# alazarteka/Self-Forcing

Measured on AMD Instinct MI355X. Metric: decoded frames/sec/node, Wan-1.3B 832x480 4-step AR rollout, higher is better.
Workload: dtype bf16

## Files before the change

include/sf_hip.h:

```cpp
#ifndef SF_HIP_H
#define SF_HIP_H

#include <stddef.h>
#include <stdint.h>

#ifdef __cplusplus
extern "C" {
#endif

#define SF_HIP_ABI_VERSION 10

int sf_abi_version(void);
const char* sf_last_error(void);

enum sf_epilogue {
  SF_EPI_BIAS = 0,
  SF_EPI_BIAS_GELU = 1,
  SF_EPI_BIAS_RESID = 2,
  SF_EPI_BIAS_GATE_RESID = 3,
  SF_EPI_F32 = 4
};

typedef struct sf_gemm_args {
  const void* a;
  const void* w;
  const void* bias;
  void* out;
  const void* resid;
  const void* gate_mod;
  const void* gate_e0;
  int64_t gate_group_stride;
  int32_t rows_per_group;
  int32_t M, N, K;
  int32_t lda, ldw, ldo, ldr;
  int32_t epilogue;
  int32_t batch;
  int64_t a_bstride, w_bstride, o_bstride, r_bstride;
  int32_t structure;
} sf_gemm_args;

enum sf_gemm_structure { SF_GEMM_AUTO = 0, SF_GEMM_T128 = 1 ,
                         SF_GEMM_PP256 = 2 ,
                         SF_GEMM_PP128 = 3 ,
                         SF_GEMM_PP224 = 4, SF_GEMM_PP192 = 5  };

int sf_gemm_bf16(const sf_gemm_args* args, void* stream);

#define SF_FP8_AMAX_PARTS 1024
int sf_quantize_fp8(const void* x, int ldx, int M, int K, int rows_per_segment, void* q_out, float* scale_out, void* stream);

int sf_gemm_fp8(const sf_gemm_args* args, const float* a_scale, int rows_per_segment, const float* w_scale, void* stream);

int sf_small_linear_fp8(const void* x, const void* w_q, const float* w_scale, const void* bias, void* out, int M, int N, int K,
                        int rows_per_segment, int act_in, int act_out, void* stream);

int sf_small_linear(const void* x, const void* w, const void* bias, void* out, int M, int N, int K,
                    int act_in, int act_out, void* stream);

int sf_sinusoid_embedding(const void* t, int t_is_int64, void* out, int n, int dim, void* stream);

int sf_layernorm_modulate(const void* x, void* out, int M, int C, float eps, const void* mod_shift,
                          const void* mod_scale, const void* e0_shift, const void* e0_scale,
                          int64_t e0_group_stride, int rows_per_group, void* stream);

int sf_layernorm_affine(const void* x, const void* weight, const void* bias, void* out, int M, int C,
                        float eps, void* stream);

int sf_rmsnorm(const void* x, int ldx, const void* weight, void* out, int ldo, int M, int C, float eps,
               void* stream);

int sf_qkv_norm_rope_cache(const void* qkv, const void* norm_q_w, const void* norm_k_w, void* q_out,
                           void* k_cache, void* v_cache, const float* rope_cos, const float* rope_sin,
                           int B, int f, int h, int w, int C, int num_heads, int64_t cache_tokens,
                           int write_start, int start_frame, float eps, void* stream);

int sf_kv_evict(void* cache, int B, int64_t cache_tokens, int row_elems, int sink, int evict, int keep,
                void* scratch, size_t scratch_bytes, void* stream);

int sf_attention(const void* q, const void* k, const void* v, void* out, int B, int H, int Lq, int Lk,
// ... 267 lines not shown
```

self-forcing_amd/_lib.py:

```python
from __future__ import annotations

import ctypes as C
import os
import subprocess
from typing import Optional

os.environ.setdefault("ROC_SIGNAL_POOL_SIZE", "1024")

_HERE = os.path.dirname(os.path.abspath(__file__))
CSRC = os.path.join(_HERE, "csrc")
LIB_PATH = os.environ.get("SF_HIP_LIB") or os.path.join(CSRC, "libsf_hip.so")

ABI_VERSION = 10
FP8_AMAX_PARTS = 1024

EPI_BIAS, EPI_BIAS_GELU, EPI_BIAS_RESID, EPI_BIAS_GATE_RESID, EPI_F32 = 0, 1, 2, 3, 4
CONV_BIAS, CONV_BIAS_RESID, CONV_BIAS_CLAMP_F32 = 0, 1, 2
VAE_MAX_STAGES = 4
ACT_NONE, ACT_SILU, ACT_GELU = 0, 1, 2
ATTN_STRUCTURES = {"auto": 0, "r64": 1, "w8": 2, "w4": 3}
CONV_STRUCTURES = {"auto": 0, "igemm": 1, "halo": 2}
GEMM_STRUCTURES = {"auto": 0, "t128": 1, "pp256": 2, "pp128": 3, "pp224": 4, "pp192": 5}


class GemmArgs(C.Structure):
    _fields_ = [
        ("a", C.c_void_p), ("w", C.c_void_p), ("bias", C.c_void_p), ("out", C.c_void_p),
        ("resid", C.c_void_p), ("gate_mod", C.c_void_p), ("gate_e0", C.c_void_p),
        ("gate_group_stride", C.c_int64), ("rows_per_group", C.c_int32),
        ("M", C.c_int32), ("N", C.c_int32), ("K", C.c_int32),
        ("lda", C.c_int32), ("ldw", C.c_int32), ("ldo", C.c_int32), ("ldr", C.c_int32),
        ("epilogue", C.c_int32), ("batch", C.c_int32),
        ("a_bstride", C.c_int64), ("w_bstride", C.c_int64), ("o_bstride", C.c_int64), ("r_bstride", C.c_int64),
        ("structure", C.c_int32),
    ]


class LayerWeights(C.Structure):
    _fields_ = [(n, C.c_void_p) for n in (
        "modulation", "norm3_w", "norm3_b", "qkv_w", "qkv_b", "norm_q_w", "norm_k_w", "o_w", "o_b",
        "cq_w", "cq_b", "ckv_w", "ckv_b", "cnorm_q_w", "cnorm_k_w", "co_w", "co_b",
        "ffn0_w", "ffn0_b", "ffn2_w", "ffn2_b")]


class LayerFp8(C.Structure):
    _fields_ = [(n, C.c_void_p) for n in (
        "qkv_q", "o_q", "cq_q", "ckv_q", "co_q", "ffn0_q", "ffn2_q",
        "qkv_s", "o_s", "cq_s", "ckv_s", "co_s", "ffn0_s", "ffn2_s")]


FP8_MODEL_LINEARS = (("text0", ("text_embedding.0",)), ("text2", ("text_embedding.2",)), ("time0", ("time_embedding.0",)),
                     ("time2", ("time_embedding.2",)), ("tproj", ("time_projection.1",)), ("head", ("head.head",)),
                     ("pose", ("pose_proj",)))
FP8_LAYER_LINEARS = (("qkv", ("self_attn.q", "self_attn.k", "self_attn.v")), ("o", ("self_attn.o",)), ("cq", ("cross_attn.q",)),
                     ("ckv", ("cross_attn.k", "cross_attn.v")), ("co", ("cross_attn.o",)), ("ffn0", ("ffn.0",)), ("ffn2", ("ffn.2",)))
# ... 70 lines not shown
        ("head_gamma", C.c_void_p), ("head_conv", VaeConv),
    ]


class VaeEncoder(C.Structure):
    _fields_ = [
        ("z_dim", C.c_int32), ("n_stages", C.c_int32), ("res_per_stage", C.c_int32),
        ("temporal_down", C.c_int32 * VAE_MAX_STAGES),
        ("latent_mean", C.c_void_p), ("latent_std", C.c_void_p), ("conv1_w", C.c_void_p), ("conv1_b", C.c_void_p),
        ("in_conv", VaeConv), ("res_host", C.POINTER(VaeResBlock)),
        ("down_conv", VaeConv * VAE_MAX_STAGES), ("time_conv", VaeConv * VAE_MAX_STAGES),
        ("mid0", VaeResBlock), ("mid2", VaeResBlock),
        ("attn_gamma", C.c_void_p), ("attn_qk_w", C.c_void_p), ("attn_qk_b", C.c_void_p),
        ("attn_v_w", C.c_void_p), ("attn_v_b", C.c_void_p), ("attn_proj_w", C.c_void_p), ("attn_proj_b", C.c_void_p),
        ("head_gamma", C.c_void_p), ("head_conv", VaeConv),
    ]


class T5Layer(C.Structure):
    _fields_ = [(n, C.c_void_p) for n in ("norm1_w", "qk_w", "v_w", "o_w", "norm2_w", "gate_w", "fc1_w", "fc2_w", "pos_emb")]


class T5Model(C.Structure):
    _fields_ = ([(n, C.c_int32) for n in ("vocab", "dim", "dim_attn", "dim_ffn", "num_heads", "num_layers", "num_buckets")]
                + [("eps", C.c_float), ("token_embedding", C.c_void_p), ("layers_host", C.POINTER(T5Layer)),
                   ("final_norm_w", C.c_void_p)])


_vp, _i, _i64, _f, _sz = C.c_void_p, C.c_int, C.c_int64, C.c_float, C.c_size_t
SIGNATURES = {
    "sf_abi_version": (C.c_int, []),
    "sf_last_error": (C.c_char_p, []),
    "sf_gemm_bf16": (C.c_int, [C.POINTER(GemmArgs), _vp]),
    "sf_small_linear": (C.c_int, [_vp, _vp, _vp, _vp, _i, _i, _i, _i, _i, _vp]),
    "sf_quantize_fp8": (C.c_int, [_vp, _i, _i, _i, _i, _vp, _vp, _vp]),
    "sf_gemm_fp8": (C.c_int, [C.POINTER(GemmArgs), _vp, _i, _vp, _vp]),
    "sf_small_linear_fp8": (C.c_int, [_vp, _vp, _vp, _vp, _vp, _i, _i, _i, _i, _i, _i, _vp]),
    "sf_sinusoid_embedding": (C.c_int, [_vp, _i, _vp, _i, _i, _vp]),
    "sf_layernorm_modulate": (C.c_int, [_vp, _vp, _i, _i, _f, _vp, _vp, _vp, _vp, _i64, _i, _vp]),
    "sf_layernorm_affine": (C.c_int, [_vp, _vp, _vp, _vp, _i, _i, _f, _vp]),
    "sf_rmsnorm": (C.c_int, [_vp, _i, _vp, _vp, _i, _i, _i, _f, _vp]),
    "sf_qkv_norm_rope_cache": (C.c_int, [_vp, _vp, _vp, _vp, _vp, _vp, _vp, _vp, _i, _i, _i, _i, _i, _i, _i64,
                                         _i, _i, _f, _vp]),
    "sf_kv_evict": (C.c_int, [_vp, _i, _i64, _i, _i, _i, _i, _vp, _sz, _vp]),
    "sf_attention": (C.c_int, [_vp, _vp, _vp, _vp, _i, _i, _i, _i, _i64, _i64, _i64, _i64, _i64, _i64, _vp]),
    "sf_attention_ex": (C.c_int, [_vp, _vp, _vp, _vp, _i, _i, _i, _i, _i64, _i64, _i64, _i64, _i64, _i64, _i, _vp]),
    "sf_patchify": (C.c_int, [_vp, _vp, _i, _i, _i, _i, _i, _vp]),
    "sf_unpatchify_x0": (C.c_int, [_vp, _vp, _vp, _i, _vp, _vp, _i, _vp, _vp, _i, _i, _i, _i, _i, _i, _vp]),
    "sf_add_noise": (C.c_int, [_vp, _vp, _vp, _i, _vp, _vp, _i, _vp, _i, _i64, _vp]),
    "sf_lincomb_bf16": (C.c_int, [_vp, C.POINTER(C.c_void_p), C.POINTER(C.c_float), _i, _i64, _vp]),
    "sf_dit_workspace_bytes": (C.c_size_t, [C.POINTER(Model), _i, _i, _i, _i, _i]),
    "sf_dit_forward": (C.c_int, [C.POINTER(Model), C.POINTER(ForwardArgs), _vp]),
    "sf_dit_forward_pair": (C.c_int, [C.POINTER(Model), C.POINTER(ForwardArgs), C.POINTER(ForwardArgs), _vp]),
    "sf_conv_igemm": (C.c_int, [C.POINTER(ConvArgs), _vp]),
    "sf_conv_pick_nt": (C.c_int, [_i]),
    "sf_rmsnorm_silu_cl": (C.c_int, [_vp, _vp, _vp, _i64, _i, _i, _vp]),
    "sf_softmax_rows": (C.c_int, [_vp, _i64, _vp, _i64, _i, _i, _i, _f, _vp]),
    "sf_vae_prepare_latent": (C.c_int, [_vp, _vp, _vp, _vp, _vp, _vp, _i, _i, _i, _i, _vp]),
    "sf_vae_state_bytes": (C.c_size_t, [C.POINTER(VaeModel), _i, _i, _i]),
    "sf_vae_scratch_bytes": (C.c_size_t, [C.POINTER(VaeModel), _i, _i, _i]),
    "sf_vae_reset": (C.c_int, [C.POINTER(VaeModel), _vp, _sz, _i, _i, _i, _vp]),
    "sf_vae_decode_frames": (C.c_int, [C.POINTER(VaeModel), _vp, _sz, _vp, _sz, _vp, _i, _i, _i, _i, _i, _i, _i, _vp, _vp]),
    "sf_vae_prepare_pixels": (C.c_int, [_vp, _i, _i64, _vp, _i, _i, _i, _i, _vp]),
    "sf_vae_finish_latent": (C.c_int, [_vp, _i, _i, _vp, _i, _vp, _vp, _vp, _vp, _i, _i, _i, _i, _vp]),
    "sf_vae_encode_state_bytes": (C.c_size_t, [C.POINTER(VaeEncoder), _i, _i, _i]),
    "sf_vae_encode_scratch_bytes": (C.c_size_t, [C.POINTER(VaeEncoder), _i, _i, _i]),
# ... 57 lines not shown
```

self-forcing_amd/csrc/gemm_bf16.hip:

```cpp
#include <type_traits>
#include "sf_common.h"
#include "../../include/sf_hip.h"

namespace {

constexpr int BM = 128, BN = 128, BK = 64;
constexpr int GEMM_THREADS = 256;
constexpr int TILE_BYTES = BM * BK * 2;
constexpr int STAGE_BYTES = 2 * TILE_BYTES;
constexpr int GEMM_LDS = 2 * STAGE_BYTES;

struct GemmP {
  const bf16_t* a;
  const bf16_t* w;
  const bf16_t* bias;
  bf16_t* out;
  const bf16_t* resid;
  const bf16_t* gate_mod;
  const bf16_t* gate_e0;
  long gate_group_stride;
  int rows_per_group;
  int M, N, K, lda, ldw, ldo, ldr;
  int tiles_m, tiles_n;
  long a_bs, w_bs, o_bs, r_bs;
// ... 139 lines not shown
      if (m0 + i >= MT) break;
      const int m = min(m_base + (m0 + i) * 16 + r16, p.M - 1);
      const bf16_t* e0row = GATE ? p.gate_e0 + (long)(m / p.rows_per_group) * p.gate_group_stride : nullptr;
#pragma unroll
      for (int nt = 0; nt < 4; ++nt) {
        rv[i][nt] = RESID ? *reinterpret_cast<const bf16x4*>(p.resid + (long)m * p.ldr + ncol[nt]) : zero4;
        ge[i][nt] = GATE ? *reinterpret_cast<const bf16x4*>(e0row + ncol[nt]) : zero4;
      }
    }
#pragma unroll
    for (int i = 0; i < MB; ++i) {
      if (m0 + i >= MT) break;
      const int row = (m0 + i) * 16 + r16;
#pragma unroll
      for (int nt = 0; nt < 4; ++nt) {
        const int col = nt * 16 + cg * 4;
        const bf16x4 o = epi_math<EPI>(acc[m0 + i][nt], bias_v[nt], gm_v[nt], ge[i][nt], rv[i][nt]);
        const int chunk = (col >> 3) ^ (row & 7);
        *reinterpret_cast<bf16x4*>(wbuf + row * 128 + (chunk << 4) + (col & 4) * 2) = o;
      }
    }
  }
  __builtin_amdgcn_s_waitcnt(0xc07f);
  const int rr = lane >> 3, ch = lane & 7;
#pragma unroll
  for (int i = 0; i < 2 * MT; ++i) {
    const int row = i * 8 + rr;
    const int m = m_base + row, n = n_base + ch * 8;
    const bf16x8 v = *reinterpret_cast<const bf16x8*>(wbuf + row * 128 + ((ch ^ (row & 7)) << 4));
    if (m < p.M && n < p.N) *reinterpret_cast<bf16x8*>(p.out + (long)m * p.ldo + n) = v;
  }
}

template <int EPI, bool F8>
__global__ __launch_bounds__(GEMM_THREADS, 2) void gemm_bf16_kernel(GemmP p) {
  extern __shared__ __attribute__((aligned(16))) char smem[];
  const int tid = threadIdx.x;
  const int lane = tid & 63;
  const int wave = __builtin_amdgcn_readfirstlane(tid >> 6);

  if (blockIdx.y) {
    const long bz = blockIdx.y;
    p.a += bz * p.a_bs; p.w += bz * p.w_bs;
    if (EPI == SF_EPI_F32) p.out = reinterpret_cast<bf16_t*>(reinterpret_cast<float*>(p.out) + bz * p.o_bs); else p.out += bz * p.o_bs;
    if (p.resid) p.resid += bz * p.r_bs;
  }
  const int nwg = gridDim.x, bid = blockIdx.x;
  const int xcd = bid & 7, q8 = nwg >> 3, r8 = nwg & 7;
  const int wg = (xcd < r8 ? xcd * (q8 + 1) : r8 * (q8 + 1) + (xcd - r8) * q8) + (bid >> 3);
  constexpr int GROUP_M = 8;
  const int width = GROUP_M * p.tiles_n;
  const int group = wg / width, first_m = group * GROUP_M;
  const int gsz = min(p.tiles_m - first_m, GROUP_M);
  const int in_group = wg - group * width;
  const int tm = first_m + in_group % gsz, tn = in_group / gsz;
  const int m0 = tm * BM, n0 = tn * BN;

  const bf16_t* a_src[4];
  const bf16_t* w_src[4];
#pragma unroll
  for (int i = 0; i < 4; ++i) {
    const int r = (wave * 4 + i) * 8 + (lane >> 3);
    const int c = (lane & 7) ^ ((r >> 1) & 7);
    const int am = min(m0 + r, p.M - 1);
    const int wn = min(n0 + r, p.N - 1);
    a_src[i] = p.a + (long)am * p.lda + c * 8;
// ... 64 lines not shown
    for (int i = 0; i < 8; ++i) {
      const int mt = i >> 1, nt0 = (i & 1) * 2;
      acc[mt][nt0] = __builtin_amdgcn_mfma_f32_16x16x32_bf16(wf0[nt0], xf0[mt], acc[mt][nt0], 0, 0, 0);
      acc[mt][nt0 + 1] = __builtin_amdgcn_mfma_f32_16x16x32_bf16(wf0[nt0 + 1], xf0[mt], acc[mt][nt0 + 1], 0, 0, 0);
      if (i < 4) {
        xf1[i] = *reinterpret_cast<const bf16x8*>(buf + x_row_off + i * 2048 + coff1);
        glds16(a_src[i] + kn, sbase + i * 1024);
      } else {
        wf1[i - 4] = *reinterpret_cast<const bf16x8*>(buf + w_row_off + (i - 4) * 2048 + coff1);
        glds16(w_src[i - 4] + kn, sbase + TILE_BYTES + (i - 4) * 1024);
      }
      __builtin_amdgcn_sched_barrier(0);
    }
#pragma unroll
    for (int mt = 0; mt < 4; ++mt)
#pragma unroll
      for (int nt = 0; nt < 4; ++nt)
        acc[mt][nt] = __builtin_amdgcn_mfma_f32_16x16x32_bf16(wf1[nt], xf1[mt], acc[mt][nt], 0, 0, 0);
    __builtin_amdgcn_sched_barrier(0);
    __syncthreads();
  }

  if constexpr (F8) fp8_scale_acc<4>(p, acc, m0 + wr * 64, n0 + wc * 64, lane);
  const int mrow = m0 + wr * 64 + (lane & 15);
  const int ncol = n0 + wc * 64 + (lane >> 4) * 4;
  if (EPI != SF_EPI_F32 && (p.N & 7) == 0 && (p.ldo & 7) == 0)
    gemm_epilogue_lds<EPI, 4>(p, acc, m0 + wr * 64, n0 + wc * 64, smem + wave * 8192, lane);
  else
    gemm_epilogue<EPI, 4>(p, acc, mrow, ncol);
}


constexpr int PP_THREADS = 512;

template <int MT>
struct PPCfg {
  static constexpr int BM = 32 * MT;
  static constexpr int A_BYTES = BM * 128;
  static constexpr int B_BYTES = 256 * 128;
  static constexpr int STAGE = A_BYTES + B_BYTES;
  static constexpr int LDS = 2 * STAGE;
  static constexpr int PA = (2 * MT + 7) / 8;
};

template <int EPI, int MT, bool F8>
__global__ __launch_bounds__(PP_THREADS) void gemm_pp_kernel(GemmP p) {
  using Cfg = PPCfg<MT>;
  constexpr int BMp = Cfg::BM, PA = Cfg::PA;
  constexpr int HQA = (MT + 1) / 2, HQB = MT / 2;
  extern __shared__ __attribute__((aligned(16))) char smem[];
  const int tid = threadIdx.x;
  const int lane = tid & 63;
  const int wave = __builtin_amdgcn_readfirstlane(tid >> 6);
  const int grp = wave >> 2, wc = wave & 3;

  const int nwg = gridDim.x, bid = blockIdx.x;
  const int xcd = bid & 7, q8 = nwg >> 3, r8 = nwg & 7;
  const int wg = (xcd < r8 ? xcd * (q8 + 1) : r8 * (q8 + 1) + (xcd - r8) * q8) + (bid >> 3);
  constexpr int GROUP_M = MT >= 6 ? 4 : 8;
  const int width = GROUP_M * p.tiles_n;
  const int group = wg / width, first_m = group * GROUP_M;
  const int gsz = min(p.tiles_m - first_m, GROUP_M);
  const int in_group = wg - group * width;
  const int tm = first_m + in_group % gsz, tn = in_group / gsz;
  const int m0 = tm * BMp, n0 = tn * 256;

  const bf16_t* a_src[2][PA];
  const bf16_t* w_src[2][2];
#pragma unroll
  for (int h = 0; h < 2; ++h) {
#pragma unroll
    for (int i = 0; i < PA; ++i) {
      const int r = h * (BMp / 2) + (wave + 8 * i) * 8 + (lane >> 3);
      const int c = (lane & 7) ^ ((r >> 1) & 7);
      a_src[h][i] = p.a + (long)min(m0 + r, p.M - 1) * p.lda + c * 8;
    }
#pragma unroll
    for (int i = 0; i < 2; ++i) {
      const int r = h * 128 + (wave + 8 * i) * 8 + (lane >> 3);
      const int c = (lane & 7) ^ ((r >> 1) & 7);
      w_src[h][i] = p.w + (long)min(n0 + r, p.N - 1) * p.ldw + c * 8;
    }
  }
  auto dma_a = [&](int h, int kt) {
    char* base = smem + (kt & 1) * Cfg::STAGE + h * (Cfg::A_BYTES / 2) + wave * 1024;
#pragma unroll
    for (int i = 0; i < PA; ++i)
      if (wave + 8 * i < 2 * MT) glds16(a_src[h][i] + kt * BK, base + i * 8192);
  };
  auto dma_b = [&](int h, int kt) {
    char* base = smem + (kt & 1) * Cfg::STAGE + Cfg::A_BYTES + h * (Cfg::B_BYTES / 2) + wave * 1024;
#pragma unroll
    for (int i = 0; i < 2; ++i) glds16(w_src[h][i] + kt * BK, base + i * 8192);
  };

  const int i16 = lane & 15, kq = lane >> 4;
  const int swz = (i16 >> 1) & 7;
  const int x_row_off = (grp * (BMp / 2) + i16) * 128;
  const int w_row_off = Cfg::A_BYTES + (wc * 64 + i16) * 128;
  const int coff[2] = {((0 + kq) ^ swz) << 4, ((4 + kq) ^ swz) << 4};

  f32x4 acc[MT][4];
#pragma unroll
  for (int i = 0; i < MT; ++i)
#pragma unroll
    for (int j = 0; j < 4; ++j) acc[i][j] = f32x4{0.f, 0.f, 0.f, 0.f};
  bf16x8 af[HQA][2], bfr[4][2];

#ifdef SF_STAMP
  unsigned long long* stamp = (EPI == SF_EPI_BIAS && p.gate_e0) ? reinterpret_cast<unsigned long long*>(const_cast<bf16_t*>(p.gate_e0)) + ((long)bid * 2 + grp) * 8 : nullptr;
  if (stamp && (tid & 255) == 0) { stamp[0] = __builtin_amdgcn_s_memtime(); stamp[4] = __builtin_amdgcn_s_memrealtime(); }
#endif
  const int nk = p.K / BK;
  dma_a(0, 0); dma_a(1, 0); dma_b(0, 0); dma_b(1, 0);
  if (nk > 1) { dma_b(0, 1); dma_b(1, 1); asm volatile("s_waitcnt vmcnt(4)" ::: "memory"); }
  else asm volatile("s_waitcnt vmcnt(0)" ::: "memory");
  __builtin_amdgcn_s_barrier();
#ifdef SF_STAMP
  if (stamp && (tid & 255) == 0) stamp[1] = __builtin_amdgcn_s_memtime();
#endif
  if (grp == 1) __builtin_amdgcn_s_barrier();

  auto end_load_segment = [&]() {
    __builtin_amdgcn_s_waitcnt(0xc07f);
    __builtin_amdgcn_sched_barrier(0);
    __builtin_amdgcn_s_barrier();
    __builtin_amdgcn_sched_barrier(0);
  };
  auto cluster = [&](auto qc, int c0) {
    constexpr int q = decltype(qc)::value, NQ = q == 0 ? HQA : HQB;
    __builtin_amdgcn_s_setprio(1);
    if constexpr (F8) {
#pragma unroll
      for (int mt = 0; mt < NQ; ++mt)
#pragma unroll
        for (int nt = 0; nt < 2; ++nt)
          acc[q * HQA + mt][c0 + nt] = mfma_f8(bfr[c0 + nt][0], bfr[c0 + nt][1], af[mt][0], af[mt][1], acc[q * HQA + mt][c0 + nt]);
    } else {
#pragma unroll
      for (int ks = 0; ks < 2; ++ks)
#pragma unroll
        for (int mt = 0; mt < NQ; ++mt)
#pragma unroll
          for (int nt = 0; nt < 2; ++nt)
            acc[q * HQA + mt][c0 + nt] = __builtin_amdgcn_mfma_f32_16x16x32_bf16(bfr[c0 + nt][ks], af[mt][ks], acc[q * HQA + mt][c0 + nt], 0, 0, 0);
    }
    __builtin_amdgcn_s_setprio(0);
    __builtin_amdgcn_sched_barrier(0);
    __builtin_amdgcn_s_barrier();
    __builtin_amdgcn_sched_barrier(0);
  };
  auto read_a = [&](const char* buf, auto qc) {
    constexpr int q = decltype(qc)::value, NQ = q == 0 ? HQA : HQB;
#pragma unroll
    for (int mt = 0; mt < NQ; ++mt)
#pragma unroll
      for (int ks = 0; ks < 2; ++ks)
        af[mt][ks] = *reinterpret_cast<const bf16x8*>(buf + x_row_off + (q * HQA + mt) * 2048 + coff[ks]);
  };
  auto read_b = [&](const char* buf, int c0) {
#pragma unroll
    for (int nt = 0; nt < 2; ++nt)
#pragma unroll
      for (int ks = 0; ks < 2; ++ks)
        bfr[c0 + nt][ks] = *reinterpret_cast<const bf16x8*>(buf + w_row_off + (c0 + nt) * 2048 + coff[ks]);
  };

  constexpr std::integral_constant<int, 0> Q0{};
  constexpr std::integral_constant<int, 1> Q1{};
  for (int kt = 0; kt < nk; ++kt) {
    const char* buf = smem + (kt & 1) * Cfg::STAGE;
    const bool more1 = kt + 1 < nk, more2 = kt + 2 < nk;
    read_a(buf, Q0);
    read_b(buf, 0);
    if (more1) dma_a(0, kt + 1);
    end_load_segment();
    cluster(Q0, 0);
    read_b(buf, 2);
    if (more1) dma_a(1, kt + 1);
    end_load_segment();
    cluster(Q0, 2);
    read_a(buf, Q1);
    if (more2) dma_b(0, kt + 2);
    end_load_segment();
    cluster(Q1, 2);
    if (more2) {
      dma_b(1, kt + 2);
      asm volatile("s_waitcnt vmcnt(4)" ::: "memory");
    } else {
      asm volatile("s_waitcnt vmcnt(0)" ::: "memory");
    }
    end_load_segment();
    cluster(Q1, 0);
  }
  if (grp == 0) __builtin_amdgcn_s_barrier();
#ifdef SF_STAMP
  if (stamp && (tid & 255) == 0) stamp[2] = __builtin_amdgcn_s_memtime();
#endif

  const int m_base = m0 + grp * (BMp / 2), n_base = n0 + wc * 64;
  if constexpr (F8) fp8_scale_acc<MT>(p, acc, m_base, n_base, lane);
  if ((p.N & 7) == 0 && (p.ldo & 7) == 0)
    gemm_epilogue_lds<EPI, MT>(p, acc, m_base, n_base, smem + wave * (MT * 2048), lane);
  else
    gemm_epilogue<EPI, MT>(p, acc, m_base + (lane & 15), n_base + (lane >> 4) * 4);
#ifdef SF_STAMP
  asm volatile("s_waitcnt vmcnt(0)" ::: "memory");
  if (stamp && (tid & 255) == 0) { stamp[3] = __builtin_amdgcn_s_memtime(); stamp[5] = __builtin_amdgcn_s_memrealtime(); }
#endif
}

constexpr int PP2_A = 128 * 128, PP2_B = 256 * 128;
constexpr int PP2_LDS = 3 * (PP2_A + PP2_B);

template <int EPI, bool F8>
__global__ __launch_bounds__(PP_THREADS) void gemm_pp2_kernel(GemmP p) {
  extern __shared__ __attribute__((aligned(16))) char smem[];
  const int tid = threadIdx.x;
  const int lane = tid & 63;
  const int wave = __builtin_amdgcn_readfirstlane(tid >> 6);
  const int grp = wave >> 2, wc = wave & 3;

  const int nwg = gridDim.x, bid = blockIdx.x;
  const int xcd = bid & 7, q8 = nwg >> 3, r8 = nwg & 7;
  const int wg = (xcd < r8 ? xcd * (q8 + 1) : r8 * (q8 + 1) + (xcd - r8) * q8) + (bid >> 3);
  constexpr int GROUP_M = 8;
  const int width = GROUP_M * p.tiles_n;
  const int group = wg / width, first_m = group * GROUP_M;
  const int gsz = min(p.tiles_m - first_m, GROUP_M);
  const int in_group = wg - group * width;
  const int tm = first_m + in_group % gsz, tn = in_group / gsz;
  const int m0 = tm * 128, n0 = tn * 256;

  const bf16_t* a_src[2];
  const bf16_t* w_src[4];
#pragma unroll
  for (int i = 0; i < 2; ++i) {
    const int r = (wave + 8 * i) * 8 + (lane >> 3);
    a_src[i] = p.a + (long)min(m0 + r, p.M - 1) * p.lda + ((lane & 7) ^ ((r >> 1) & 7)) * 8;
  }
#pragma unroll
  for (int i = 0; i < 4; ++i) {
// ... 95 lines not shown

  const int m_base = m0 + grp * 64, n_base = n0 + wc * 64;
  if constexpr (F8) fp8_scale_acc<4>(p, acc, m_base, n_base, lane);
  if ((p.N & 7) == 0 && (p.ldo & 7) == 0)
    gemm_epilogue_lds<EPI, 4>(p, acc, m_base, n_base, smem + wave * 8192, lane);
  else
    gemm_epilogue<EPI, 4>(p, acc, m_base + (lane & 15), n_base + (lane >> 4) * 4);
}

template <int EPI, bool F8>
int launch_pp2(GemmP& p, hipStream_t s) {
  static bool attr = false;
  if (!attr) {
    (void)hipFuncSetAttribute(reinterpret_cast<const void*>(&gemm_pp2_kernel<EPI, F8>), hipFuncAttributeMaxDynamicSharedMemorySize, PP2_LDS);
    attr = true;
  }
  p.tiles_m = (p.M + 127) / 128;
  p.tiles_n = (p.N + 255) / 256;
  hipLaunchKernelGGL((gemm_pp2_kernel<EPI, F8>), dim3(p.tiles_m * p.tiles_n), dim3(PP_THREADS), PP2_LDS, s, p);
  return 0;
}

template <bool F8>
int launch_pp2_epi(GemmP& p, int epilogue, hipStream_t s) {
  switch (epilogue) {
    case SF_EPI_BIAS: return launch_pp2<SF_EPI_BIAS, F8>(p, s);
    case SF_EPI_BIAS_GELU: return launch_pp2<SF_EPI_BIAS_GELU, F8>(p, s);
    case SF_EPI_BIAS_RESID: return launch_pp2<SF_EPI_BIAS_RESID, F8>(p, s);
    case SF_EPI_BIAS_GATE_RESID: return launch_pp2<SF_EPI_BIAS_GATE_RESID, F8>(p, s);
    default: return -1;
  }
}

template <int EPI, int MT, bool F8>
int launch_pp(GemmP& p, hipStream_t s) {
  using Cfg = PPCfg<MT>;
  static bool attr = false;
  if (!attr) {
    (void)hipFuncSetAttribute(reinterpret_cast<const void*>(&gemm_pp_kernel<EPI, MT, F8>), hipFuncAttributeMaxDynamicSharedMemorySize, Cfg::LDS);
    attr = true;
  }
  p.tiles_m = (p.M + Cfg::BM - 1) / Cfg::BM;
  p.tiles_n = (p.N + 255) / 256;
  hipLaunchKernelGGL((gemm_pp_kernel<EPI, MT, F8>), dim3(p.tiles_m * p.tiles_n), dim3(PP_THREADS), Cfg::LDS, s, p);
  return 0;
}

template <int MT, bool F8>
int launch_pp_epi(GemmP& p, int epilogue, hipStream_t s) {
  switch (epilogue) {
    case SF_EPI_BIAS: return launch_pp<SF_EPI_BIAS, MT, F8>(p, s);
    case SF_EPI_BIAS_GELU: return launch_pp<SF_EPI_BIAS_GELU, MT, F8>(p, s);
    case SF_EPI_BIAS_RESID: return launch_pp<SF_EPI_BIAS_RESID, MT, F8>(p, s);
    case SF_EPI_BIAS_GATE_RESID: return launch_pp<SF_EPI_BIAS_GATE_RESID, MT, F8>(p, s);
    default: return -1;
  }
}

int check_args(const sf_gemm_args* a, const char* name, int bk) {
  SF_CHECK(a != nullptr, "%s: null args", name);
  SF_CHECK(a->M > 0 && a->N > 0 && a->K > 0, "%s: empty problem M=%d N=%d K=%d", name, a->M, a->N, a->K);
  SF_CHECK(a->K % bk == 0, "%s: K=%d must be a multiple of %d", name, a->K, bk);
  SF_CHECK(a->N % 4 == 0, "%s: N=%d must be a multiple of 4", name, a->N);
  SF_CHECK(a->lda % (bk / 8) == 0 && a->ldw % (bk / 8) == 0 && a->ldo % 4 == 0, "%s: lda/ldw must be multiples of %d, ldo of 4", name, bk / 8);
  SF_CHECK(a->lda >= a->K && a->ldw >= a->K && a->ldo >= a->N, "%s: leading dimension too small", name);
  SF_CHECK(a->a && a->w && a->out, "%s: null tensor", name);
  SF_CHECK(((uintptr_t)a->a % 16 == 0) && ((uintptr_t)a->w % 16 == 0) && ((uintptr_t)a->out % 8 == 0), "%s: misaligned tensor", name);
  if (a->epilogue == SF_EPI_BIAS_RESID || a->epilogue == SF_EPI_BIAS_GATE_RESID) {
    SF_CHECK(a->resid != nullptr && a->ldr >= a->N && a->ldr % 4 == 0, "%s: residual epilogue needs resid/ldr", name);
  }
  if (a->epilogue == SF_EPI_BIAS_GATE_RESID) {
    SF_CHECK(a->gate_mod && a->gate_e0 && a->rows_per_group > 0, "%s: gate epilogue needs gate_mod/gate_e0/rows_per_group", name);
  }
  SF_CHECK(a->structure >= SF_GEMM_AUTO && a->structure <= SF_GEMM_PP192, "%s: unknown structure %d", name, a->structure);
  return 0;
}

template <bool F8>
int run_gemm(const sf_gemm_args* a, GemmP& p, const char* name, hipStream_t s) {
  int st = a->structure;
  const int nk = p.K / BK;
  const bool pp_ok = a->batch <= 1 && a->epilogue != SF_EPI_F32 && nk >= 2;
  if (st == SF_GEMM_AUTO) {
    st = SF_GEMM_T128;
    if (pp_ok && a->M >= 1024 && a->N >= 1024 && a->K >= 512) {
      static const struct { int st, rows; double rel; } cand[] = {
          {SF_GEMM_PP256, 256, 1.00}, {SF_GEMM_PP224, 224, 1.02}, {SF_GEMM_PP192, 192, 1.05}, {SF_GEMM_PP128, 128, 1.14}};
      const long tn = (a->N + 255) / 256;
      double best = 1e30;
      for (const auto& c : cand) {
        const long tiles = (long)((a->M + c.rows - 1) / c.rows) * tn;
        const double cost = (double)((tiles + 255) / 256) * (c.rows / 256.0 * c.rel + 0.04);
        if (cost < best - 1e-9) { best = cost; st = c.st; }
      }
    }
  }
  const bool is_pp = st == SF_GEMM_PP256 || st == SF_GEMM_PP224 || st == SF_GEMM_PP192 || st == SF_GEMM_PP128;
  if (is_pp && !pp_ok) st = SF_GEMM_T128;
  else if (is_pp) {
    const int rc = st == SF_GEMM_PP256 ? launch_pp_epi<8, F8>(p, a->epilogue, s)
                 : st == SF_GEMM_PP224 ? launch_pp_epi<7, F8>(p, a->epilogue, s)
                 : st == SF_GEMM_PP192 ? launch_pp_epi<6, F8>(p, a->epilogue, s) : launch_pp2_epi<F8>(p, a->epilogue, s);
    SF_CHECK(rc == 0, "%s: unknown epilogue %d", name, a->epilogue);
    SF_HIP_LAUNCH_CHECK(name);
    return 0;
  }
  const int batch = a->batch > 1 ? a->batch : 1;
  p.a_bs = a->a_bstride; p.w_bs = a->w_bstride; p.o_bs = a->o_bstride; p.r_bs = a->r_bstride;
  SF_CHECK(batch == 1 || (a->a_bstride % 8 == 0 && a->w_bstride % 8 == 0 && a->o_bstride % 4 == 0 && a->r_bstride % 4 == 0),
           "%s: batch strides must keep 16-byte (operands) / 8-byte (output) alignment", name);
  const dim3 grid(p.tiles_m * p.tiles_n, batch), block(GEMM_THREADS);
  switch (a->epilogue) {
    case SF_EPI_BIAS: hipLaunchKernelGGL((gemm_bf16_kernel<SF_EPI_BIAS, F8>), grid, block, GEMM_LDS, s, p); break;
    case SF_EPI_BIAS_GELU: hipLaunchKernelGGL((gemm_bf16_kernel<SF_EPI_BIAS_GELU, F8>), grid, block, GEMM_LDS, s, p); break;
    case SF_EPI_BIAS_RESID: hipLaunchKernelGGL((gemm_bf16_kernel<SF_EPI_BIAS_RESID, F8>), grid, block, GEMM_LDS, s, p); break;
    case SF_EPI_BIAS_GATE_RESID: hipLaunchKernelGGL((gemm_bf16_kernel<SF_EPI_BIAS_GATE_RESID, F8>), grid, block, GEMM_LDS, s, p); break;
    case SF_EPI_F32:
      if constexpr (F8) {
        SF_CHECK(false, "%s: the raw fp32 epilogue is bf16-only", name);
      } else {
        SF_CHECK((uintptr_t)a->out % 16 == 0, "%s: fp32 output must be 16-byte aligned", name);
        hipLaunchKernelGGL((gemm_bf16_kernel<SF_EPI_F32, false>), grid, block, GEMM_LDS, s, p);
      }
      break;
    default: SF_CHECK(false, "%s: unknown epilogue %d", name, a->epilogue);
  }
  SF_HIP_LAUNCH_CHECK(name);
  return 0;
}

void fill_params(const sf_gemm_args* a, GemmP& p, int unit) {
  p.a = (const bf16_t*)a->a; p.w = (const bf16_t*)a->w; p.bias = (const bf16_t*)a->bias;
  p.out = (bf16_t*)a->out; p.resid = (const bf16_t*)a->resid;
  p.gate_mod = (const bf16_t*)a->gate_mod; p.gate_e0 = (const bf16_t*)a->gate_e0;
  p.gate_group_stride = a->gate_group_stride; p.rows_per_group = a->rows_per_group;
  p.M = a->M; p.N = a->N; p.K = a->K / unit; p.lda = a->lda / unit; p.ldw = a->ldw / unit; p.ldo = a->ldo; p.ldr = a->ldr;
  p.tiles_n = (a->N + BN - 1) / BN;
  p.tiles_m = (a->M + BM - 1) / BM;
  p.a_scale = nullptr; p.w_scale = nullptr; p.rows_per_seg = 1;
}

}

extern "C" int sf_gemm_bf16(const sf_gemm_args* a, void* stream) {
  if (const int rc = check_args(a, "sf_gemm_bf16", BK)) return rc;
  GemmP p;
  fill_params(a, p, 1);
  return run_gemm<false>(a, p, "sf_gemm_bf16", (hipStream_t)stream);
}

extern "C" int sf_gemm_fp8(const sf_gemm_args* a, const float* a_scale, int rows_per_segment, const float* w_scale, void* stream) {
  if (const int rc = check_args(a, "sf_gemm_fp8", 2 * BK)) return rc;
  SF_CHECK(a->batch <= 1, "sf_gemm_fp8: batched products are bf16-only");
  SF_CHECK(a_scale && w_scale && rows_per_segment > 0, "sf_gemm_fp8: needs a_scale, w_scale and rows_per_segment > 0");
  SF_CHECK((uintptr_t)w_scale % 16 == 0, "sf_gemm_fp8: w_scale must be 16-byte aligned");
  GemmP p;
  fill_params(a, p, 2);
  p.a_scale = a_scale; p.w_scale = w_scale; p.rows_per_seg = rows_per_segment;
  return run_gemm<true>(a, p, "sf_gemm_fp8", (hipStream_t)stream);
}
```

Before: 96.18.

## Add persistent tile-loop PP GEMM that prefetches next tile during epilogue

Adds a persistent variant of the ping-pong GEMM kernel that launches at most 256 workgroups and loops over output tiles. Each workgroup issues the first loads for its next tile before running the current tile's epilogue, which goes through separate LDS scratch regions. Stores are left outstanding and waited on with adjusted vmcnt counts. This is meant to hide epilogue and tile-startup latency and avoid extra waves when the tile count exceeds the grid. The cost is a larger LDS footprint, more complex counter-based synchronisation, and a serial tile walk per workgroup. Auto-selection switches to the loop form whenever the chosen PP config has more than 256 tiles.

New measurement: 97.07 (median of 6 runs). No clear change (+0.9%).

```diff
diff --git a/include/sf_hip.h b/include/sf_hip.h
--- a/include/sf_hip.h
+++ b/include/sf_hip.h
@@ -42,9 +42,12 @@
 enum sf_gemm_structure { SF_GEMM_AUTO = 0, SF_GEMM_T128 = 1 ,
                          SF_GEMM_PP256 = 2 ,
                          SF_GEMM_PP128 = 3 ,
-                         SF_GEMM_PP224 = 4, SF_GEMM_PP192 = 5  };
+                         SF_GEMM_PP224 = 4, SF_GEMM_PP192 = 5 ,
+                         SF_GEMM_PP256_LOOP = 6, SF_GEMM_PP224_LOOP = 7, SF_GEMM_PP192_LOOP = 8  };
 
 int sf_gemm_bf16(const sf_gemm_args* args, void* stream);
+
+int sf_gemm_pp_loop_lds_map(int row_tiles, int32_t out[7]);
 
 #define SF_FP8_AMAX_PARTS 1024
 int sf_quantize_fp8(const void* x, int ldx, int M, int K, int rows_per_segment, void* q_out, float* scale_out, void* stream);
diff --git a/self-forcing_amd/_lib.py b/self-forcing_amd/_lib.py
--- a/self-forcing_amd/_lib.py
+++ b/self-forcing_amd/_lib.py
@@ -20,7 +20,8 @@
 ACT_NONE, ACT_SILU, ACT_GELU = 0, 1, 2
 ATTN_STRUCTURES = {"auto": 0, "r64": 1, "w8": 2, "w4": 3}
 CONV_STRUCTURES = {"auto": 0, "igemm": 1, "halo": 2}
-GEMM_STRUCTURES = {"auto": 0, "t128": 1, "pp256": 2, "pp128": 3, "pp224": 4, "pp192": 5}
+GEMM_STRUCTURES = {"auto": 0, "t128": 1, "pp256": 2, "pp128": 3, "pp224": 4, "pp192": 5,
+                   "pp256_loop": 6, "pp224_loop": 7, "pp192_loop": 8}
 
 
 class GemmArgs(C.Structure):
@@ -157,6 +158,7 @@
     "sf_abi_version": (C.c_int, []),
     "sf_last_error": (C.c_char_p, []),
     "sf_gemm_bf16": (C.c_int, [C.POINTER(GemmArgs), _vp]),
+    "sf_gemm_pp_loop_lds_map": (C.c_int, [_i, C.POINTER(C.c_int32)]),
     "sf_small_linear": (C.c_int, [_vp, _vp, _vp, _vp, _i, _i, _i, _i, _i, _vp]),
     "sf_quantize_fp8": (C.c_int, [_vp, _i, _i, _i, _i, _vp, _vp, _vp]),
     "sf_gemm_fp8": (C.c_int, [C.POINTER(GemmArgs), _vp, _i, _vp, _vp]),
diff --git a/self-forcing_amd/csrc/gemm_bf16.hip b/self-forcing_amd/csrc/gemm_bf16.hip
--- a/self-forcing_amd/csrc/gemm_bf16.hip
+++ b/self-forcing_amd/csrc/gemm_bf16.hip
@@ -195,6 +195,74 @@
   }
 }
 
+template <int EPI, int MT, class RequestNext>
+__device__ __forceinline__ void gemm_epilogue_lds_loop(const GemmP& p, f32x4 (&acc)[MT][4], const bf16x4 (&bias_v)[4], int m_base, int n_base,
+                                                       char* wbuf, int lane, RequestNext&& request_next) {
+  const int r16 = lane & 15, cg = lane >> 4;
+  constexpr bool GATE = EPI == SF_EPI_BIAS_GATE_RESID;
+  constexpr bool RESID = EPI == SF_EPI_BIAS_RESID || EPI == SF_EPI_BIAS_GATE_RESID;
+  constexpr int HALF = 8 * MT;
+  constexpr int SPLIT = (MT + 1) / 2;
+  const bf16x4 zero4 = {(bf16_t)0.f, (bf16_t)0.f, (bf16_t)0.f, (bf16_t)0.f};
+  int ncol[4];
+  bf16x4 gm_v[4];
+#pragma unroll
+  for (int nt = 0; nt < 4; ++nt) {
+    ncol[nt] = min(n_base + nt * 16 + cg * 4, p.N - 4);
+    gm_v[nt] = GATE ? *reinterpret_cast<const bf16x4*>(p.gate_mod + ncol[nt]) : zero4;
+  }
+  bf16x4 rv[MT][4], ge[MT][4];
+  auto load_rows = [&](auto lo, auto hi) {
+#pragma unroll
+    for (int mt = decltype(lo)::value; mt < decltype(hi)::value; ++mt) {
+      const int m = min(m_base + mt * 16 + r16, p.M - 1);
+      const bf16_t* e0row = GATE ? p.gate_e0 + (long)(m / p.rows_per_group) * p.gate_group_stride : nullptr;
+#pragma unroll
+      for (int nt = 0; nt < 4; ++nt) {
+        rv[mt][nt] = RESID ? *reinterpret_cast<const bf16x4*>(p.resid + (long)m * p.ldr + ncol[nt]) : zero4;
+        ge[mt][nt] = GATE ? *reinterpret_cast<const bf16x4*>(e0row + ncol[nt]) : zero4;
+      }
+    }
+  };
+  constexpr std::integral_constant<int, 0> I0{};
+  constexpr std::integral_constant<int, SPLIT> IS{};
+  constexpr std::integral_constant<int, MT> IM{};
+  if (!GATE) load_rows(I0, IM);
+#pragma unroll
+  for (int nt = 0; nt < 4; ++nt) asm volatile("" ::"v"(bias_v[nt]));
+  request_next();
+  const int rr = lane >> 3, ch = lane & 7;
+#pragma unroll
+  for (int ps = 0; ps < 2; ++ps) {
+    if (GATE) {
+      if (ps == 0) load_rows(I0, IS); else load_rows(IS, IM);
+    }
+#pragma unroll
+    for (int mt = ps * (MT / 2); mt < (ps == 0 ? SPLIT : MT); ++mt) {
+      const int srow = mt * 16 + r16 - ps * HALF;
+#pragma unroll
+      for (int nt = 0; nt < 4; ++nt) {
+        const int col = nt * 16 + cg * 4;
+        const bf16x4 o = epi_math<EPI>(acc[mt][nt], bias_v[nt], gm_v[nt], ge[mt][nt], rv[mt][nt]);
+        const int chunk = (col >> 3) ^ (srow & 7);
+        if ((unsigned)srow < (unsigned)HALF) *reinterpret_cast<bf16x4*>(wbuf + srow * 128 + (chunk << 4) + (col & 4) * 2) = o;
+      }
+    }
+    __builtin_amdgcn_s_waitcnt(0xc07f);
+    bf16x8 v[MT];
+#pragma unroll
+    for (int i = 0; i < MT; ++i) {
+      const int srow = i * 8 + rr;
+      v[i] = *reinterpret_cast<const bf16x8*>(wbuf + srow * 128 + ((ch ^ (srow & 7)) << 4));
+    }
+#pragma unroll
+    for (int i = 0; i < MT; ++i) {
+      const int m = m_base + ps * HALF + i * 8 + rr, n = n_base + ch * 8;
+      if (m < p.M && n < p.N) *reinterpret_cast<bf16x8*>(p.out + (long)m * p.ldo + n) = v[i];
+    }
+  }
+}
+
 template <int EPI, bool F8>
 __global__ __launch_bounds__(GEMM_THREADS, 2) void gemm_bf16_kernel(GemmP p) {
   extern __shared__ __attribute__((aligned(16))) char smem[];
@@ -325,6 +393,8 @@
 
 
 constexpr int PP_THREADS = 512;
+constexpr int PP_LOOP_WGS = 256;
+constexpr bool PP_AUTO_TILE_LOOP = true;
 
 template <int MT>
 struct PPCfg {
@@ -334,9 +404,11 @@
   static constexpr int STAGE = A_BYTES + B_BYTES;
   static constexpr int LDS = 2 * STAGE;
   static constexpr int PA = (2 * MT + 7) / 8;
+  static constexpr int SCRATCH = MT * 1024;
+  static constexpr int LDS_LOOP = LDS + 4 * SCRATCH;
 };
 
-template <int EPI, int MT, bool F8>
+template <int EPI, int MT, bool F8, bool LOOP>
 __global__ __launch_bounds__(PP_THREADS) void gemm_pp_kernel(GemmP p) {
   using Cfg = PPCfg<MT>;
   constexpr int BMp = Cfg::BM, PA = Cfg::PA;
@@ -347,34 +419,43 @@
   const int wave = __builtin_amdgcn_readfirstlane(tid >> 6);
   const int grp = wave >> 2, wc = wave & 3;
 
-  const int nwg = gridDim.x, bid = blockIdx.x;
-  const int xcd = bid & 7, q8 = nwg >> 3, r8 = nwg & 7;
-  const int wg = (xcd < r8 ? xcd * (q8 + 1) : r8 * (q8 + 1) + (xcd - r8) * q8) + (bid >> 3);
+  const int nwg = LOOP ? p.tiles_m * p.tiles_n : gridDim.x, bid = blockIdx.x;
   constexpr int GROUP_M = MT >= 6 ? 4 : 8;
-  const int width = GROUP_M * p.tiles_n;
-  const int group = wg / width, first_m = group * GROUP_M;
-  const int gsz = min(p.tiles_m - first_m, GROUP_M);
-  const int in_group = wg - group * width;
-  const int tm = first_m + in_group % gsz, tn = in_group / gsz;
-  const int m0 = tm * BMp, n0 = tn * 256;
+  int m0, n0;
+  auto tile_origin = [&](int t) {
+    const int xcd = t & 7, q8 = nwg >> 3, r8 = nwg & 7;
+    const int wg = (xcd < r8 ? xcd * (q8 + 1) : r8 * (q8 + 1) + (xcd - r8) * q8) + (t >> 3);
+    const int width = GROUP_M * p.tiles_n;
+    const int group = wg / width, first_m = group * GROUP_M;
+    const int gsz = min(p.tiles_m - first_m, GROUP_M);
+    const int in_group = wg - group * width;
+    m0 = (first_m + in_group % gsz) * BMp;
+    n0 = (in_group / gsz) * 256;
+  };
 
   const bf16_t* a_src[2][PA];
   const bf16_t* w_src[2][2];
-#pragma unroll
-  for (int h = 0; h < 2; ++h) {
-#pragma unroll
-    for (int i = 0; i < PA; ++i) {
-      const int r = h * (BMp / 2) + (wave + 8 * i) * 8 + (lane >> 3);
-      const int c = (lane & 7) ^ ((r >> 1) & 7);
-      a_src[h][i] = p.a + (long)min(m0 + r, p.M - 1) * p.lda + c * 8;
-    }
-#pragma unroll
-    for (int i = 0; i < 2; ++i) {
-      const int r = h * 128 + (wave + 8 * i) * 8 + (lane >> 3);
-      const int c = (lane & 7) ^ ((r >> 1) & 7);
-      w_src[h][i] = p.w + (long)min(n0 + r, p.N - 1) * p.ldw + c * 8;
-    }
-  }
+  auto set_sources = [&]() {
+    int ln = lane;
+    if (LOOP) asm volatile("" : "+v"(ln));
+#pragma unroll
+    for (int h = 0; h < 2; ++h) {
+#pragma unroll
+      for (int i = 0; i < PA; ++i) {
+        const int r = h * (BMp / 2) + (wave + 8 * i) * 8 + (ln >> 3);
+        const int c = (ln & 7) ^ ((r >> 1) & 7);
+        a_src[h][i] = p.a + (long)min(m0 + r, p.M - 1) * p.lda + c * 8;
+      }
+#pragma unroll
+      for (int i = 0; i < 2; ++i) {
+        const int r = h * 128 + (wave + 8 * i) * 8 + (ln >> 3);
+        const int c = (ln & 7) ^ ((r >> 1) & 7);
+        w_src[h][i] = p.w + (long)min(n0 + r, p.N - 1) * p.ldw + c * 8;
+      }
+    }
+  };
+  tile_origin(bid);
+  set_sources();
   auto dma_a = [&](int h, int kt) {
     char* base = smem + (kt & 1) * Cfg::STAGE + h * (Cfg::A_BYTES / 2) + wave * 1024;
 #pragma unroll
@@ -385,6 +466,11 @@
     char* base = smem + (kt & 1) * Cfg::STAGE + Cfg::A_BYTES + h * (Cfg::B_BYTES / 2) + wave * 1024;
 #pragma unroll
     for (int i = 0; i < 2; ++i) glds16(w_src[h][i] + kt * BK, base + i * 8192);
+  };
+  const int nk = p.K / BK;
+  auto first_requests = [&]() {
+    dma_a(0, 0); dma_a(1, 0); dma_b(0, 0); dma_b(1, 0);
+    if (nk > 1) { dma_b(0, 1); dma_b(1, 1); }
   };
 
   const int i16 = lane & 15, kq = lane >> 4;
@@ -394,25 +480,13 @@
   const int coff[2] = {((0 + kq) ^ swz) << 4, ((4 + kq) ^ swz) << 4};
 
   f32x4 acc[MT][4];
-#pragma unroll
-  for (int i = 0; i < MT; ++i)
-#pragma unroll
-    for (int j = 0; j < 4; ++j) acc[i][j] = f32x4{0.f, 0.f, 0.f, 0.f};
   bf16x8 af[HQA][2], bfr[4][2];
 
 #ifdef SF_STAMP
   unsigned long long* stamp = (EPI == SF_EPI_BIAS && p.gate_e0) ? reinterpret_cast<unsigned long long*>(const_cast<bf16_t*>(p.gate_e0)) + ((long)bid * 2 + grp) * 8 : nullptr;
-  if (stamp && (tid & 255) == 0) { stamp[0] = __builtin_amdgcn_s_memtime(); stamp[4] = __builtin_amdgcn_s_memrealtime(); }
+  if (!LOOP && stamp && (tid & 255) == 0) { stamp[0] = __builtin_amdgcn_s_memtime(); stamp[4] = __builtin_amdgcn_s_memrealtime(); }
 #endif
-  const int nk = p.K / BK;
-  dma_a(0, 0); dma_a(1, 0); dma_b(0, 0); dma_b(1, 0);
-  if (nk > 1) { dma_b(0, 1); dma_b(1, 1); asm volatile("s_waitcnt vmcnt(4)" ::: "memory"); }
-  else asm volatile("s_waitcnt vmcnt(0)" ::: "memory");
-  __builtin_amdgcn_s_barrier();
-#ifdef SF_STAMP
-  if (stamp && (tid & 255) == 0) stamp[1] = __builtin_amdgcn_s_memtime();
-#endif
-  if (grp == 1) __builtin_amdgcn_s_barrier();
+  first_requests();
 
   auto end_load_segment = [&]() {
     __builtin_amdgcn_s_waitcnt(0xc07f);
@@ -461,46 +535,105 @@
 
   constexpr std::integral_constant<int, 0> Q0{};
   constexpr std::integral_constant<int, 1> Q1{};
-  for (int kt = 0; kt < nk; ++kt) {
-    const char* buf = smem + (kt & 1) * Cfg::STAGE;
-    const bool more1 = kt + 1 < nk, more2 = kt + 2 < nk;
-    read_a(buf, Q0);
-    read_b(buf, 0);
-    if (more1) dma_a(0, kt + 1);
-    end_load_segment();
-    cluster(Q0, 0);
-    read_b(buf, 2);
-    if (more1) dma_a(1, kt + 1);
-    end_load_segment();
-    cluster(Q0, 2);
-    read_a(buf, Q1);
-    if (more2) dma_b(0, kt + 2);
-    end_load_segment();
-    cluster(Q1, 2);
-    if (more2) {
-      dma_b(1, kt + 2);
-      asm volatile("s_waitcnt vmcnt(4)" ::: "memory");
+  constexpr int NST = 2 * MT;
+  const int ntiles = nwg;
+  bool stores_pending = false;
+  for (int tile = bid;;) {
+#ifdef SF_STAMP
+    const bool stamp_on = stamp && (tid & 255) == 0 && (!LOOP || tile == bid + (int)gridDim.x);
+    if (LOOP && stamp_on) { stamp[0] = __builtin_amdgcn_s_memtime(); stamp[4] = __builtin_amdgcn_s_memrealtime(); }
+#endif
+#pragma unroll
+    for (int i = 0; i < MT; ++i)
+#pragma unroll
+      for (int j = 0; j < 4; ++j) acc[i][j] = f32x4{0.f, 0.f, 0.f, 0.f};
+    if (LOOP && stores_pending) {
+      if (nk > 1) asm volatile("s_waitcnt vmcnt(%0)" ::"n"(4 + NST) : "memory");
+      else asm volatile("s_waitcnt vmcnt(%0)" ::"n"(NST) : "memory");
     } else {
-      asm volatile("s_waitcnt vmcnt(0)" ::: "memory");
-    }
-    end_load_segment();
-    cluster(Q1, 0);
-  }
-  if (grp == 0) __builtin_amdgcn_s_barrier();
+      if (nk > 1) asm volatile("s_waitcnt vmcnt(4)" ::: "memory");
+      else asm volatile("s_waitcnt vmcnt(0)" ::: "memory");
+    }
+    __builtin_amdgcn_s_barrier();
 #ifdef SF_STAMP
-  if (stamp && (tid & 255) == 0) stamp[2] = __builtin_amdgcn_s_memtime();
+    if (stamp_on) stamp[1] = __builtin_amdgcn_s_memtime();
 #endif
-
-  const int m_base = m0 + grp * (BMp / 2), n_base = n0 + wc * 64;
-  if constexpr (F8) fp8_scale_acc<MT>(p, acc, m_base, n_base, lane);
-  if ((p.N & 7) == 0 && (p.ldo & 7) == 0)
-    gemm_epilogue_lds<EPI, MT>(p, acc, m_base, n_base, smem + wave * (MT * 2048), lane);
-  else
-    gemm_epilogue<EPI, MT>(p, acc, m_base + (lane & 15), n_base + (lane >> 4) * 4);
+    if (grp == 1) __builtin_amdgcn_s_barrier();
+    bf16x4 bias_v[4];
+    if constexpr (LOOP) {
+#pragma unroll
+      for (int nt = 0; nt < 4; ++nt) {
+        bias_v[nt] = bf16x4{(bf16_t)0.f, (bf16_t)0.f, (bf16_t)0.f, (bf16_t)0.f};
+        if (p.bias) bias_v[nt] = *reinterpret_cast<const bf16x4*>(p.bias + min(n0 + wc * 64 + nt * 16 + (lane >> 4) * 4, p.N - 4));
+      }
+    }
+
+    for (int kt = 0; kt < nk; ++kt) {
+      const char* buf = smem + (kt & 1) * Cfg::STAGE;
+      const bool more1 = kt + 1 < nk, more2 = kt + 2 < nk;
+      read_a(buf, Q0);
+      read_b(buf, 0);
+      if (more1) dma_a(0, kt + 1);
+      end_load_segment();
+      cluster(Q0, 0);
+      read_b(buf, 2);
+      if (more1) dma_a(1, kt + 1);
+      end_load_segment();
+      cluster(Q0, 2);
+      read_a(buf, Q1);
+      if (more2) dma_b(0, kt + 2);
+      end_load_segment();
+      cluster(Q1, 2);
+      if (more2) {
+        dma_b(1, kt + 2);
+        asm volatile("s_waitcnt vmcnt(4)" ::: "memory");
+      } else {
+        asm volatile("s_waitcnt vmcnt(0)" ::: "memory");
+      }
+      end_load_segment();
+      cluster(Q1, 0);
+    }
+    if (grp == 0) __builtin_amdgcn_s_barrier();
 #ifdef SF_STAMP
-  asm volatile("s_waitcnt vmcnt(0)" ::: "memory");
-  if (stamp && (tid & 255) == 0) { stamp[3] = __builtin_amdgcn_s_memtime(); stamp[5] = __builtin_amdgcn_s_memrealtime(); }
+    if (stamp_on) stamp[2] = __builtin_amdgcn_s_memtime();
 #endif
+
+    const int m_base = m0 + grp * (BMp / 2), n_base = n0 + wc * 64;
+    if constexpr (F8) fp8_scale_acc<MT>(p, acc, m_base, n_base, lane);
+    if constexpr (!LOOP) {
+      if ((p.N & 7) == 0 && (p.ldo & 7) == 0)
+        gemm_epilogue_lds<EPI, MT>(p, acc, m_base, n_base, smem + wave * (MT * 2048), lane);
+      else
+        gemm_epilogue<EPI, MT>(p, acc, m_base + (lane & 15), n_base + (lane >> 4) * 4);
+    } else {
+      const int next = tile + gridDim.x;
+      auto request_next = [&]() {
+        __builtin_amdgcn_sched_barrier(0);
+        if (next < ntiles) {
+          tile_origin(next);
+          set_sources();
+          first_requests();
+        }
+        __builtin_amdgcn_sched_barrier(0);
+      };
+      char* scratch = smem + (grp == 0 ? Cfg::STAGE : 2 * Cfg::STAGE) + wc * Cfg::SCRATCH;
+      if ((p.N & 7) == 0 && (p.ldo & 7) == 0) {
+        gemm_epilogue_lds_loop<EPI, MT>(p, acc, bias_v, m_base, n_base, scratch, lane, request_next);
+        stores_pending = m_base + 16 * MT <= p.M && n_base + 64 <= p.N;
+      } else {
+        request_next();
+        gemm_epilogue<EPI, MT>(p, acc, m_base + (lane & 15), n_base + (lane >> 4) * 4);
+        stores_pending = false;
+      }
+    }
+#ifdef SF_STAMP
+    if (!LOOP) asm volatile("s_waitcnt vmcnt(0)" ::: "memory");
+    if (stamp_on) { stamp[3] = __builtin_amdgcn_s_memtime(); stamp[5] = __builtin_amdgcn_s_memrealtime(); }
+#endif
+    if (!LOOP) break;
+    tile += gridDim.x;
+    if (tile >= ntiles) break;
+  }
 }
 
 constexpr int PP2_A = 128 * 128, PP2_B = 256 * 128;
@@ -662,27 +795,30 @@
   }
 }
 
-template <int EPI, int MT, bool F8>
+template <int EPI, int MT, bool F8, bool LOOP>
 int launch_pp(GemmP& p, hipStream_t s) {
   using Cfg = PPCfg<MT>;
+  constexpr int lds = LOOP ? Cfg::LDS_LOOP : Cfg::LDS;
+  static_assert(lds <= 160 * 1024, "a workgroup's LDS");
   static bool attr = false;
   if (!attr) {
-    (void)hipFuncSetAttribute(reinterpret_cast<const void*>(&gemm_pp_kernel<EPI, MT, F8>), hipFuncAttributeMaxDynamicSharedMemorySize, Cfg::LDS);
+    (void)hipFuncSetAttribute(reinterpret_cast<const void*>(&gemm_pp_kernel<EPI, MT, F8, LOOP>), hipFuncAttributeMaxDynamicSharedMemorySize, lds);
     attr = true;
   }
   p.tiles_m = (p.M + Cfg::BM - 1) / Cfg::BM;
   p.tiles_n = (p.N + 255) / 256;
-  hipLaunchKernelGGL((gemm_pp_kernel<EPI, MT, F8>), dim3(p.tiles_m * p.tiles_n), dim3(PP_THREADS), Cfg::LDS, s, p);
+  const int tiles = p.tiles_m * p.tiles_n;
+  hipLaunchKernelGGL((gemm_pp_kernel<EPI, MT, F8, LOOP>), dim3(LOOP ? min(tiles, PP_LOOP_WGS) : tiles), dim3(PP_THREADS), lds, s, p);
   return 0;
 }
 
-template <int MT, bool F8>
+template <int MT, bool F8, bool LOOP>
 int launch_pp_epi(GemmP& p, int epilogue, hipStream_t s) {
   switch (epilogue) {
-    case SF_EPI_BIAS: return launch_pp<SF_EPI_BIAS, MT, F8>(p, s);
-    case SF_EPI_BIAS_GELU: return launch_pp<SF_EPI_BIAS_GELU, MT, F8>(p, s);
-    case SF_EPI_BIAS_RESID: return launch_pp<SF_EPI_BIAS_RESID, MT, F8>(p, s);
-    case SF_EPI_BIAS_GATE_RESID: return launch_pp<SF_EPI_BIAS_GATE_RESID, MT, F8>(p, s);
+    case SF_EPI_BIAS: return launch_pp<SF_EPI_BIAS, MT, F8, LOOP>(p, s);
+    case SF_EPI_BIAS_GELU: return launch_pp<SF_EPI_BIAS_GELU, MT, F8, LOOP>(p, s);
+    case SF_EPI_BIAS_RESID: return launch_pp<SF_EPI_BIAS_RESID, MT, F8, LOOP>(p, s);
+    case SF_EPI_BIAS_GATE_RESID: return launch_pp<SF_EPI_BIAS_GATE_RESID, MT, F8, LOOP>(p, s);
     default: return -1;
   }
 }
@@ -702,7 +838,7 @@
   if (a->epilogue == SF_EPI_BIAS_GATE_RESID) {
     SF_CHECK(a->gate_mod && a->gate_e0 && a->rows_per_group > 0, "%s: gate epilogue needs gate_mod/gate_e0/rows_per_group", name);
   }
-  SF_CHECK(a->structure >= SF_GEMM_AUTO && a->structure <= SF_GEMM_PP192, "%s: unknown structure %d", name, a->structure);
+  SF_CHECK(a->structure >= SF_GEMM_AUTO && a->structure <= SF_GEMM_PP192_LOOP, "%s: unknown structure %d", name, a->structure);
   return 0;
 }
 
@@ -718,19 +854,29 @@
           {SF_GEMM_PP256, 256, 1.00}, {SF_GEMM_PP224, 224, 1.02}, {SF_GEMM_PP192, 192, 1.05}, {SF_GEMM_PP128, 128, 1.14}};
       const long tn = (a->N + 255) / 256;
       double best = 1e30;
+      long loop_tiles = 0;
       for (const auto& c : cand) {
         const long tiles = (long)((a->M + c.rows - 1) / c.rows) * tn;
         const double cost = (double)((tiles + 255) / 256) * (c.rows / 256.0 * c.rel + 0.04);
-        if (cost < best - 1e-9) { best = cost; st = c.st; }
-      }
-    }
-  }
+        if (cost < best - 1e-9) { best = cost; st = c.st; loop_tiles = tiles; }
+      }
+      if (PP_AUTO_TILE_LOOP && st != SF_GEMM_PP128 && loop_tiles > PP_LOOP_WGS)
+        st = st == SF_GEMM_PP256 ? SF_GEMM_PP256_LOOP : st == SF_GEMM_PP224 ? SF_GEMM_PP224_LOOP : SF_GEMM_PP192_LOOP;
+    }
+  }
+  const bool loop_form = st >= SF_GEMM_PP256_LOOP;
+  if (loop_form) st = st == SF_GEMM_PP256_LOOP ? SF_GEMM_PP256 : st == SF_GEMM_PP224_LOOP ? SF_GEMM_PP224 : SF_GEMM_PP192;
   const bool is_pp = st == SF_GEMM_PP256 || st == SF_GEMM_PP224 || st == SF_GEMM_PP192 || st == SF_GEMM_PP128;
   if (is_pp && !pp_ok) st = SF_GEMM_T128;
   else if (is_pp) {
-    const int rc = st == SF_GEMM_PP256 ? launch_pp_epi<8, F8>(p, a->epilogue, s)
-                 : st == SF_GEMM_PP224 ? launch_pp_epi<7, F8>(p, a->epilogue, s)
-                 : st == SF_GEMM_PP192 ? launch_pp_epi<6, F8>(p, a->epilogue, s) : launch_pp2_epi<F8>(p, a->epilogue, s);
+    int rc;
+    if (loop_form)
+      rc = st == SF_GEMM_PP256 ? launch_pp_epi<8, F8, true>(p, a->epilogue, s)
+         : st == SF_GEMM_PP224 ? launch_pp_epi<7, F8, true>(p, a->epilogue, s) : launch_pp_epi<6, F8, true>(p, a->epilogue, s);
+    else
+      rc = st == SF_GEMM_PP256 ? launch_pp_epi<8, F8, false>(p, a->epilogue, s)
+         : st == SF_GEMM_PP224 ? launch_pp_epi<7, F8, false>(p, a->epilogue, s)
+         : st == SF_GEMM_PP192 ? launch_pp_epi<6, F8, false>(p, a->epilogue, s) : launch_pp2_epi<F8>(p, a->epilogue, s);
     SF_CHECK(rc == 0, "%s: unknown epilogue %d", name, a->epilogue);
     SF_HIP_LAUNCH_CHECK(name);
     return 0;
@@ -772,6 +918,21 @@
 
 }
 
+extern "C" int sf_gemm_pp_loop_lds_map(int row_tiles, int32_t out[7]) {
+  auto fill = [&](auto cfg) {
+    using Cfg = decltype(cfg);
+    out[0] = Cfg::A_BYTES; out[1] = Cfg::B_BYTES; out[2] = Cfg::STAGE; out[3] = Cfg::SCRATCH;
+    out[4] = Cfg::STAGE; out[5] = 2 * Cfg::STAGE; out[6] = Cfg::LDS_LOOP;
+    return 0;
+  };
+  switch (row_tiles) {
+    case 8: return fill(PPCfg<8>{});
+    case 7: return fill(PPCfg<7>{});
+    case 6: return fill(PPCfg<6>{});
+    default: return -1;
+  }
+}
+
 extern "C" int sf_gemm_bf16(const sf_gemm_args* a, void* stream) {
   if (const int rc = check_args(a, "sf_gemm_bf16", BK)) return rc;
   GemmP p;
```
